# NVIDIA/makani

Measured on AMD Instinct MI355X. Metric: SFNO train samples/sec at 721x1440x73ch, higher is better.
Workload: dtype bf16; 1 GPU; sfno_sc3_layers8_edim384; grid=721x1440, channels=73, global_batch=1, parallelism=dp1, spectral_arithmetic=x3, multistep_count=1, multistep_checkpoint=False, launch=hipGraph replay of the captured step, channel_gemm=hip (csrc/conv1x1.hip)

## Files before the change

makani_amd/csrc/conv1x1.hip:

```cpp
#include <stdlib.h>
#include <type_traits>

#include "common.h"
#include "conv1x1_plan.h"

#ifndef MK_ASTAT_DIAG
#define MK_ASTAT_DIAG 0
#endif
#if MK_ASTAT_DIAG
__device__ unsigned long long g_astat_diag[16];
#define MK_AS_STAMP(k)                                              \
    do {                                                            \
        const unsigned long long t_ = __builtin_readcyclecounter(); \
        dg[k] += t_ - tprev;                                        \
        tprev = t_;                                                 \
    } while (0)
#else
#define MK_AS_STAMP(k)
#endif

namespace {

typedef __bf16 bf16x8 __attribute__((ext_vector_type(8)));
typedef __attribute__((address_space(3))) s16x4 lds_s16x4;
// ... 185 lines not shown
        }
    };

    const int s = lane & 15, g1 = (lane >> 4) & 1;
    const int a_off = (wm * WM + l31) * PA + lh * 8;
    const int b_off = (lh * 8 + (s >> 2)) * PB + wn * WN + g1 * 16 + (s & 3) * 4;
    auto compute = [&](int buf) {
        const u16* Ab = As + buf * BM * PA;
        const u16* Bb = Bs + buf * BK * PB;
#pragma unroll
        for (int ks = 0; ks < BK / 16; ++ks) {
            bf16x8 af[TM], bfr[TN];
#pragma unroll
            for (int i = 0; i < TM; ++i)
                af[i] = __builtin_bit_cast(bf16x8, *reinterpret_cast<const s16x8*>(Ab + a_off + i * 32 * PA + ks * 16));
#pragma unroll
            for (int j = 0; j < TN; ++j) {
                const u16* q0 = Bb + b_off + (ks * 16) * PB + j * 32;
                const s16x4 lo = __builtin_amdgcn_ds_read_tr16_b64_v4i16((lds_s16x4*)(q0));
                const s16x4 hi = __builtin_amdgcn_ds_read_tr16_b64_v4i16((lds_s16x4*)(q0 + 4 * PB));
                const s16x8 v = {lo[0], lo[1], lo[2], lo[3], hi[0], hi[1], hi[2], hi[3]};
                bfr[j] = __builtin_bit_cast(bf16x8, v);
            }
#pragma unroll
            for (int i = 0; i < TM; ++i)
#pragma unroll
                for (int j = 0; j < TN; ++j)
                    acc[i][j] = __builtin_amdgcn_mfma_f32_32x32x16_bf16(af[i], bfr[j], acc[i][j], 0, 0, 0);
        }
    };

    const int nk = (p.K + BK - 1) / BK;
    load_tiles(ra[0], rb[0], 0);
    if constexpr (DEPTH == 2) {
        if (nk > 1) load_tiles(ra[1], rb[1], BK);
        store_tiles(ra[0], rb[0], 0);
        __syncthreads();
        for (int kt = 0; kt < nk; kt += 2) {
            if (kt + 2 < nk) load_tiles(ra[0], rb[0], (kt + 2) * BK);
            compute(0);
            if (kt + 1 < nk) store_tiles(ra[1], rb[1], 1);
            __syncthreads();
            if (kt + 1 >= nk) break;
            if (kt + 3 < nk) load_tiles(ra[1], rb[1], (kt + 3) * BK);
            compute(1);
            if (kt + 2 < nk) store_tiles(ra[0], rb[0], 0);
            __syncthreads();
        }
    } else if constexpr (LDSB == 2) {
        store_tiles(ra[0], rb[0], 0);
        __syncthreads();
        for (int kt = 0; kt < nk; ++kt) {
            if (kt + 1 < nk) load_tiles(ra[0], rb[0], (kt + 1) * BK);
            compute(kt & 1);
            if (kt + 1 < nk) store_tiles(ra[0], rb[0], (kt & 1) ^ 1);
            __syncthreads();
        }
    } else {
        store_tiles(ra[0], rb[0], 0);
        __syncthreads();
        for (int kt = 0; kt < nk; ++kt) {
            if (kt + 1 < nk) load_tiles(ra[0], rb[0], (kt + 1) * BK);
            compute(0);
            __syncthreads();
            if (kt + 1 < nk) {
                store_tiles(ra[0], rb[0], 0);
                __syncthreads();
            }
        }
    }

    const long long plane = (long long)b * p.M * p.N;
    const bool vec_ok = (p.N % 8) == 0;
#pragma unroll
    for (int half = 0; half < 2; ++half) {
        if (wm == half) {
#pragma unroll
            for (int i = 0; i < TM; ++i)
#pragma unroll
                for (int j = 0; j < TN; ++j)
#pragma unroll
                    for (int r = 0; r < 16; ++r) {
                        const int row = i * 32 + (r & 3) + 8 * (r >> 2) + 4 * lh;
                        Es[row * PE + wn * WN + j * 32 + l31] = acc[i][j][r];
                    }
        }
        __syncthreads();
        for (int f = tid; f < WM * (BN / 8); f += NT) {
            const int row = f / (BN / 8), c = f % (BN / 8);
            const int m = m0 + half * WM + row;
            const long long n = n0 + c * 8;
            if (m >= p.M || n >= p.N) continue;
            const float bv = p.bias ? p.bias[m] : 0.f;
            const long long o = plane + (long long)m * p.N + n;
            float v[8];
            const float4 e0 = *reinterpret_cast<const float4*>(Es + row * PE + c * 8);
            const float4 e1 = *reinterpret_cast<const float4*>(Es + row * PE + c * 8 + 4);
            v[0] = e0.x + bv, v[1] = e0.y + bv, v[2] = e0.z + bv, v[3] = e0.w + bv;
            v[4] = e1.x + bv, v[5] = e1.y + bv, v[6] = e1.z + bv, v[7] = e1.w + bv;
            const bool full = vec_ok && n + 8 <= p.N;
            auto put = [&](u16* dst, const float* x) {
                if (full) {
                    uint4 u;
                    u.x = pack_bf16x2(x[0], x[1]);
                    u.y = pack_bf16x2(x[2], x[3]);
                    u.z = pack_bf16x2(x[4], x[5]);
                    u.w = pack_bf16x2(x[6], x[7]);
                    *reinterpret_cast<uint4*>(dst + o) = u;
                } else {
                    for (int e = 0; e < 8 && n + e < p.N; ++e) dst[o + e] = f32_to_bf16(x[e]);
                }
            };
            auto get = [&](const u16* src, float* x) {
                if (full) {
                    const uint4 u = ld16(src + o);
                    const uint32_t w[4] = {u.x, u.y, u.z, u.w};
#pragma unroll
                    for (int e = 0; e < 4; ++e) {
                        x[2 * e] = __uint_as_float(w[e] << 16);
                        x[2 * e + 1] = __uint_as_float(w[e] & 0xffff0000u);
                    }
                } else {
                    for (int e = 0; e < 8; ++e) x[e] = (n + e < p.N) ? bf16_to_f32(src[o + e]) : 0.f;
                }
            };
            if (p.act) {
                if (p.Ypre) put(p.Ypre, v);
#pragma unroll
                for (int e = 0; e < 8; ++e) v[e] = gelu_f(v[e]);
            }
            if (p.G) {
                float g[8];
                get(p.G, g);
#pragma unroll
                for (int e = 0; e < 8; ++e) v[e] *= gelu_grad_f(g[e]);
            }
            if (p.R) {
                float rr[8];
                get(p.R, rr);
#pragma unroll
                for (int e = 0; e < 8; ++e) v[e] += rr[e];
            }
            put(p.Y, v);
        }
        __syncthreads();
    }
}

template <int TM>
__global__ __launch_bounds__(512, 2) void conv_nn_ring_kernel(const ConvNN p, int tilesM, long long tilesN, long long ntiles) {
#if defined(__HIP_DEVICE_COMPILE__)
    constexpr int TN = 2;
    constexpr int BM = 2 * TM * 32, BN = 256, BK = 64;
    constexpr int ASZ = BM * 128, XSZ = BK * BN * 2, STAGE = ASZ + XSZ;
    constexpr int NIA = BM / 64, NIX = 4, NI = NIA + NIX;
    constexpr int EROWS = 64;
    __shared__ __attribute__((aligned(1024))) unsigned char smem[2 * STAGE + EROWS * 512];
    unsigned char* const stg = smem + 2 * STAGE;

    const int tid = threadIdx.x, lane = tid & 63, wave = tid >> 6;
    const int wm = wave >> 2, wn = wave & 3;
    const int l31 = lane & 31, lh = lane >> 5;
    const int nk = (p.K + BK - 1) / BK;
    const unsigned rowbytes = (unsigned)(p.N * 2);

    const int ca_log = (lane & 7) ^ ((((wave & 1) << 2) + (lane >> 4)) & 7);
    const int kx3 = (2 * (wave & 1) + (lane >> 5)) & 3;
    const int cx_log = (lane & 31) ^ (kx3 << 2);
    unsigned voffx[NIX];
#pragma unroll
    for (int j = 0; j < NIX; ++j) voffx[j] = (unsigned)(2 * (wave + 8 * j) + (lane >> 5)) * rowbytes + (unsigned)cx_log * 16u;
    const v4i_t rsA = make_rsrc_n(p.A, (unsigned)((long long)p.M * p.lda * 2));
    const unsigned lds_w = lds_addr(smem) + __builtin_amdgcn_readfirstlane(wave) * 1024;

    const int swa = (l31 >> 1) & 7;
    int aoff[4];
#pragma unroll
    for (int ks = 0; ks < 4; ++ks) aoff[ks] = (wm * TM * 32 + l31) * 128 + (((ks * 2 + lh) ^ swa) * 16);
    const int s15 = lane & 15, g1 = (lane >> 4) & 1;
    int xoff[TN];
#pragma unroll
    for (int j = 0; j < TN; ++j)
        xoff[j] = ASZ + (lh * 8 + (s15 >> 2)) * 512 + ((((wn * TN + j) ^ ((s15 >> 2) & 3)) * 4 + g1 * 2 + ((s15 & 3) >> 1)) * 16) + (s15 & 1) * 8;

    const long long first = xcd_remap(blockIdx.x, gridDim.x);
    unsigned voffa[NIA];
    unsigned voffx_t[NIX];
    const u16* xb = p.X;
    int m0 = 0, bcur = -1;
    long long n0 = 0;

    auto setup_tile = [&](long long t) {
        const int tm = (int)(t % tilesM);
        const long long tnb = t / tilesM;
        const int b = (int)(tnb / tilesN);
        m0 = tm * BM;
        n0 = (tnb % tilesN) * BN;
        if (b != bcur) {
            bcur = b;
            xb = p.X + (long long)b * p.K * p.N;
        }
#pragma unroll
        for (int i = 0; i < NIA; ++i) {
            const int row = min(m0 + (wave + 8 * i) * 8 + (lane >> 3), p.M - 1);
            voffa[i] = (unsigned)row * (unsigned)(p.lda * 2) + (unsigned)ca_log * 16u;
        }
        const int cmax = (int)((min(p.N, n0 + BN) - n0) / 8) - 1;
#pragma unroll
        for (int j = 0; j < NIX; ++j) voffx_t[j] = voffx[j] - (unsigned)max(0, cx_log - cmax) * 16u;
    };
    auto issue = [&](int kt, int stage) {
        const unsigned dst = lds_w + stage * STAGE;
        const unsigned soffa = (unsigned)(kt * BK * 2);
        const v4i_t rsX = make_rsrc_n(xb + (long long)kt * BK * p.N, (unsigned)min(BK, p.K - kt * BK) * rowbytes);
        const unsigned soffx = (unsigned)__builtin_amdgcn_readfirstlane((int)(unsigned)(n0 * 2));
        if constexpr (NIA == 4) dma4<8192>(dst, rsA, soffa, voffa[0], voffa[1], voffa[2], voffa[3]);
        else dma3<8192>(dst, rsA, soffa, voffa[0], voffa[1], voffa[2]);
        dma4<8192>(dst + ASZ, rsX, soffx, voffx_t[0], voffx_t[1], voffx_t[2], voffx_t[3]);
    };

    f32x16 acc[TM][TN];
    auto compute = [&](int stage) {
        const unsigned char* sb = smem + stage * STAGE;
#pragma unroll
        for (int ks = 0; ks < 4; ++ks) {
            bf16x8 af[TM], xf[TN];
#pragma unroll
            for (int i = 0; i < TM; ++i) af[i] = __builtin_bit_cast(bf16x8, *reinterpret_cast<const s16x8*>(sb + aoff[ks] + i * 4096));
#pragma unroll
            for (int j = 0; j < TN; ++j) {
                const unsigned char* q0 = sb + xoff[j] + ks * 16 * 512;
                const s16x4 lo = __builtin_amdgcn_ds_read_tr16_b64_v4i16((lds_s16x4*)(q0));
                const s16x4 hi = __builtin_amdgcn_ds_read_tr16_b64_v4i16((lds_s16x4*)(q0 + 4 * 512));
                const s16x8 v = {lo[0], lo[1], lo[2], lo[3], hi[0], hi[1], hi[2], hi[3]};
                xf[j] = __builtin_bit_cast(bf16x8, v);
            }
#pragma unroll
            for (int i = 0; i < TM; ++i)
#pragma unroll
                for (int j = 0; j < TN; ++j)
                    acc[i][j] = __builtin_amdgcn_mfma_f32_32x32x16_bf16(xf[j], af[i], acc[i][j], 0, 0, 0);
        }
    };

    long long t = first;
    if (t < ntiles) {
        setup_tile(t);
        issue(0, 0);
        if (nk > 1) issue(1, 1);
    }
    for (; t < ntiles; t += gridDim.x) {
#pragma unroll
        for (int i = 0; i < TM; ++i)
#pragma unroll
            for (int j = 0; j < TN; ++j)
#pragma unroll
                for (int r = 0; r < 16; ++r) acc[i][j][r] = 0.f;
        const int cm0 = m0;
        const long long cn0 = n0;
        const int cb = bcur;
        float bvr[TM];
#pragma unroll
        for (int i = 0; i < TM; ++i) {
            const int mrow = cm0 + (wm * TM + i) * 32 + l31;
            bvr[i] = (p.bias && mrow < p.M) ? p.bias[mrow] : 0.f;
        }
#pragma unroll
        for (int i = 0; i < TM; ++i) asm volatile("" : "+v"(bvr[i]));
        for (int kt = 0; kt < nk; ++kt) {
            if (kt == 0 || kt + 1 >= nk) wait_vmcnt<0>(); else wait_vmcnt<NI>();
            __builtin_amdgcn_s_barrier();
            compute(kt & 1);
            asm volatile("s_waitcnt lgkmcnt(0)" ::: "memory");
            __builtin_amdgcn_s_barrier();
            if (kt + 2 < nk) issue(kt + 2, kt & 1);
        }
        const bool have_next = t + gridDim.x < ntiles;
        const bool epi_loads = p.G || p.R;
        if (have_next) setup_tile(t + gridDim.x);
        if (have_next && !epi_loads) {
            issue(0, 0);
            if (nk > 1) issue(1, 1);
        }

        const long long plane = (long long)cb * p.M * p.N;
#pragma unroll
        for (int i = 0; i < TM; ++i) {
            long long off[4];
            bool live[4];
            uint4 gq[4], rq[4];
#pragma unroll
            for (int u4 = 0; u4 < 4; ++u4) {
                const int idx = tid + 512 * u4;
                const int row = idx >> 5, ch = idx & 31;
                const int m = cm0 + ((row >> 5) * TM + i) * 32 + (row & 31);
                const long long n = cn0 + ch * 8;
                live[u4] = m < p.M && n < p.N;
                off[u4] = plane + (long long)m * p.N + n;
                gq[u4] = rq[u4] = make_uint4(0, 0, 0, 0);
                if (live[u4] && p.G) gq[u4] = ld16(p.G + off[u4]);
                if (live[u4] && p.R) rq[u4] = ld16(p.R + off[u4]);
            }
            const float bv = bvr[i];
            const int lrow = wm * 32 + l31;
#pragma unroll
            for (int j = 0; j < TN; ++j)
#pragma unroll
                for (int q = 0; q < 4; ++q) {
                    const int px = (wn * TN + j) * 32 + 8 * q + 4 * lh;
                    uint2 u;
                    u.x = pack_bf16x2(acc[i][j][4 * q] + bv, acc[i][j][4 * q + 1] + bv);
                    u.y = pack_bf16x2(acc[i][j][4 * q + 2] + bv, acc[i][j][4 * q + 3] + bv);
                    *reinterpret_cast<uint2*>(stg + lrow * 512 + (((px >> 3) ^ (lrow & 15)) * 16) + ((px >> 2) & 1) * 8) = u;
                }
            asm volatile("s_waitcnt lgkmcnt(0)" ::: "memory");
            __builtin_amdgcn_s_barrier();
            if (epi_loads) {
#pragma unroll
                for (int u4 = 0; u4 < 4; ++u4) {
                    asm volatile("" : "+v"(gq[u4].x), "+v"(gq[u4].y), "+v"(gq[u4].z), "+v"(gq[u4].w));
                    asm volatile("" : "+v"(rq[u4].x), "+v"(rq[u4].y), "+v"(rq[u4].z), "+v"(rq[u4].w));
                }
                if (i == TM - 1 && have_next) {
                    issue(0, 0);
                    if (nk > 1) issue(1, 1);
                }
            }
#pragma unroll
            for (int u4 = 0; u4 < 4; ++u4) {
                const int idx = tid + 512 * u4;
                const int row = idx >> 5, ch = idx & 31;
                const uint4 raw = *reinterpret_cast<const uint4*>(stg + row * 512 + ((ch ^ (row & 15)) * 16));
                if (live[u4]) {
                    const long long o = off[u4];
                    if (!p.act && !p.G && !p.R) {
                        mk_st16(p.Y + o, raw, p.nt);
                    } else {
                        if (p.act && p.Ypre) mk_st16(p.Ypre + o, raw, p.nt);
                        const uint32_t w[4] = {raw.x, raw.y, raw.z, raw.w};
                        float v[8];
#pragma unroll
                        for (int e = 0; e < 4; ++e) {
                            v[2 * e] = __uint_as_float(w[e] << 16);
                            v[2 * e + 1] = __uint_as_float(w[e] & 0xffff0000u);
                        }
                        if (p.act) {
                            gelu_fast_n<8>(v);
                        }
                        if (p.G) {
                            const uint32_t gw[4] = {gq[u4].x, gq[u4].y, gq[u4].z, gq[u4].w};
#pragma unroll
                            for (int e = 0; e < 4; ++e) {
                                const float ga2[2] = {__uint_as_float(gw[e] << 16), __uint_as_float(gw[e] & 0xffff0000u)};
                                float gd2[2];
                                gelu_grad_fast_n<2>(ga2, gd2);
                                v[2 * e] *= gd2[0];
                                v[2 * e + 1] *= gd2[1];
                            }
                        }
                        if (p.R) {
                            const uint32_t rw[4] = {rq[u4].x, rq[u4].y, rq[u4].z, rq[u4].w};
#pragma unroll
                            for (int e = 0; e < 4; ++e) {
                                v[2 * e] += __uint_as_float(rw[e] << 16);
                                v[2 * e + 1] += __uint_as_float(rw[e] & 0xffff0000u);
                            }
                        }
                        uint4 out;
                        out.x = pack_bf16x2(v[0], v[1]);
                        out.y = pack_bf16x2(v[2], v[3]);
                        out.z = pack_bf16x2(v[4], v[5]);
                        out.w = pack_bf16x2(v[6], v[7]);
                        mk_st16(p.Y + o, out, p.nt);
                    }
                }
            }
            asm volatile("s_waitcnt lgkmcnt(0)" ::: "memory");
            __builtin_amdgcn_s_barrier();
        }
    }
#endif
}

template <int N_> __device__ __forceinline__ void wait_vmcnt_le() {
    if constexpr (N_ <= 63) wait_vmcnt<N_>(); else wait_vmcnt<63>();
}

template <int TM, int KCH, bool PRE, bool EPI_LOADS, int KS = 24>
__global__ __launch_bounds__(256, (KS < 24 && !EPI_LOADS) ? 2 : 1) void conv_nn_astat_kernel(const ConvNN p, int slabs, long long tilesN) {
#if defined(__HIP_DEVICE_COMPILE__)
    constexpr bool SMALLK = KS < 24;
    static_assert(KS == 24 || (KS * 16 <= KCH && KCH % 32 == 0), "small K: one chunk per pixel tile");
    constexpr int TN = 2;
    constexpr int BM = 4 * TM * 32, BN = 64, NT_ = 256;
    constexpr int CH = KCH * 128;
    constexpr int NCH = SMALLK ? 1 : 384 / KCH;
    constexpr int K4 = KS / NCH;
    constexpr int ROUNDS_ = TM;
    constexpr int EBYTES = EPI_LOADS ? ROUNDS_ * 128 * 128 : 0;
    constexpr int NSLOT = SMALLK ? (EPI_LOADS ? 8 : 5) : (EPI_LOADS ? (144 * 1024 - EBYTES) : 128 * 1024) / CH;
    constexpr int NP = KCH / 32;
    constexpr int ROUNDS = TM;
    constexpr int NSTORE = ROUNDS * 4 * (PRE ? 2 : 1);
    constexpr int EPIECES = EPI_LOADS ? ROUNDS * 4 : 0;
    constexpr int LOOK = SMALLK ? ((PRE || EPI_LOADS) ? 2 : 3) : (KCH == 64 ? 8 : ((NP * 4 + 2 * NSTORE <= 63) ? 5 : 4));
    constexpr int SMALLK_EPI_WAIT = NSTORE + (LOOK - 1) * (EPIECES + NP + NSTORE);
    static_assert(!(SMALLK && EPI_LOADS) || SMALLK_EPI_WAIT <= 63, "vmcnt is a 6-bit counter");
    constexpr int NEPI_MAX = (LOOK + NCH - 1) / NCH;
    static_assert(LOOK <= NSLOT - 1, "a slot is refilled only after every wave has left it");
    static_assert(EPI_LOADS || NP * (LOOK - 1) + NEPI_MAX * NSTORE <= 63, "vmcnt is a 6-bit counter");
    __shared__ __attribute__((aligned(1024))) unsigned char smem[NSLOT * CH + EBYTES + 128 * 128];
    unsigned char* const ebuf = smem + NSLOT * CH;
    unsigned char* const stg = ebuf + EBYTES;

    const int tid = threadIdx.x, lane = tid & 63, wave = tid >> 6;
    const bool nt_st = p.nt != 0;
    const int l31 = lane & 31, lh = lane >> 5;
    const int s15 = lane & 15, g1 = (lane >> 4) & 1;
#if MK_ASTAT_DIAG
    unsigned long long dg[8] = {0, 0, 0, 0, 0, 0, 0, 0};
    unsigned long long tprev = __builtin_readcyclecounter();
    const unsigned long long tstart = tprev;
#endif

    const int vid = xcd_remap(blockIdx.x, gridDim.x);
    const int slab = vid % slabs;
    const int pstride = gridDim.x / slabs;
    const int pfirst = vid / slabs;
    const int tilesN32 = (int)tilesN;
    const int my_tiles = pfirst < tilesN32 ? (tilesN32 - pfirst + pstride - 1) / pstride : 0;
    const int cb = blockIdx.y;
    const int m_base = slab * BM + wave * (TM * 32);
    const unsigned nbytes = (unsigned)(p.N * 2);

    bf16x8 af[TM][KS];
#pragma unroll
    for (int i = 0; i < TM; ++i) {
        const int row = min(m_base + i * 32 + l31, p.M - 1);
        const u16* src = p.A + (long long)row * p.lda + lh * 8;
#pragma unroll
        for (int ks = 0; ks < KS; ++ks) af[i][ks] = __builtin_bit_cast(bf16x8, ld16(src + ks * 16));
    }
    float bvr[TM];
#pragma unroll
    for (int i = 0; i < TM; ++i) {
        const int mrow = m_base + i * 32 + l31;
        bvr[i] = (p.bias && mrow < p.M) ? p.bias[mrow] : 0.f;
    }
#pragma unroll
    for (int i = 0; i < TM; ++i) {
#pragma unroll
        for (int ks = 0; ks < KS; ++ks) asm volatile("" : "+v"(af[i][ks]));
        asm volatile("" : "+v"(bvr[i]));
    }

    const unsigned lds0 = lds_addr(smem) + __builtin_amdgcn_readfirstlane(wave) * (NP * 1024);
    unsigned vx[NP];
    const int cxl = (lane & 7) ^ ((((lane >> 3) >> 1) & 1) << 2);
#pragma unroll
    for (int q = 0; q < NP; ++q) vx[q] = (unsigned)((wave * NP + q) * 8 + (lane >> 3)) * nbytes + (unsigned)cxl * 16u;
    const v4i_t rsX = SMALLK ? make_rsrc_n(p.X + (long long)cb * p.K * p.N, (unsigned)p.K * nbytes) : make_rsrc(p.X + (long long)cb * p.K * p.N);
    const unsigned kstride = (unsigned)KCH * nbytes;
    int i_pt = pfirst, i_kc = 0, i_slot = 0;
    auto issue_next = [&]() {
        const unsigned n0b = (unsigned)i_pt * (BN * 2);
        const int cmax = min(7, (int)((nbytes - n0b) / 16) - 1);
        const unsigned soff = (unsigned)__builtin_amdgcn_readfirstlane((int)((unsigned)i_kc * kstride + n0b));
        const unsigned back = (unsigned)max(0, cxl - cmax) * 16u;
        if constexpr (NP == 2) dma2<1024>(lds0 + (unsigned)i_slot * CH, rsX, soff, vx[0] - back, vx[1] - back);
        else if constexpr (NP == 3) dma3<1024>(lds0 + (unsigned)i_slot * CH, rsX, soff, vx[0] - back, vx[1] - back, vx[2] - back);
        else dma4<1024>(lds0 + (unsigned)i_slot * CH, rsX, soff, vx[0] - back, vx[1] - back, vx[2] - back, vx[3] - back);
        i_slot = i_slot + 1 == NSLOT ? 0 : i_slot + 1;
        if (++i_kc == NCH) {
            i_kc = 0;
            i_pt += pstride;
        }
    };

    const u16* const eop = p.G ? p.G : p.R;
    const v4i_t rsE = make_rsrc(EPI_LOADS ? (const void*)(eop + (long long)cb * p.M * p.N) : (const void*)p.X);
    const unsigned ldsE = lds_addr(ebuf) + __builtin_amdgcn_readfirstlane(wave) * 4096;
    auto issue_epi = [&](long long cn0) {
        const unsigned n0b = (unsigned)(cn0 * 2);
        const int cmax = min(7, (int)((nbytes - n0b) / 16) - 1);
        const unsigned col = (unsigned)min(lane & 7, cmax) * 16u;
        const unsigned soff = (unsigned)__builtin_amdgcn_readfirstlane((int)n0b);
#pragma unroll
        for (int i = 0; i < (EPI_LOADS ? ROUNDS_ : 0); ++i) {
            unsigned v[4];
#pragma unroll
            for (int q = 0; q < 4; ++q) v[q] = (unsigned)min(m_base + i * 32 + q * 8 + (lane >> 3), p.M - 1) * nbytes + col;
            dma4<1024>(ldsE + (unsigned)i * 16384u, rsE, soff, v[0], v[1], v[2], v[3]);
        }
    };

    int xoff[TN];
#pragma unroll
    for (int j = 0; j < TN; ++j) {
        const int kk = lh * 8 + (s15 >> 2);
        const int chunk = (j * 4 + g1 * 2 + ((s15 & 3) >> 1)) ^ (((kk >> 1) & 1) << 2);
        xoff[j] = kk * 128 + chunk * 16 + (s15 & 1) * 8;
    }

    const int nchunks = my_tiles * NCH;
    MK_AS_STAMP(7);
    for (int c = 0; c < LOOK && c < nchunks; ++c) issue_next();
    int c_slot = 0;

    f32x16 acc[TM][TN];
    const long long plane0 = (long long)cb * p.M * p.N;
    const __amdgpu_buffer_rsrc_t rsY = __builtin_amdgcn_make_buffer_rsrc((void*)(p.Y + plane0), 0, 0x80000000u, 0x00020000);
    const __amdgpu_buffer_rsrc_t rsP = __builtin_amdgcn_make_buffer_rsrc((void*)((PRE ? p.Ypre : p.Y) + plane0), 0, 0x80000000u, 0x00020000);

    for (int ts = 0; ts < my_tiles; ++ts) {
#pragma unroll
        for (int i = 0; i < TM; ++i)
#pragma unroll
            for (int j = 0; j < TN; ++j)
#pragma unroll
                for (int r = 0; r < 16; ++r) acc[i][j][r] = 0.f;
        const long long cn0 = (long long)(pfirst + ts * pstride) * BN;

#pragma unroll
        for (int kc = 0; kc < NCH; ++kc) {
            const int c = ts * NCH + kc;
            const int nfull = (LOOK - kc + NCH - 1) / NCH;
            if (c + LOOK > nchunks) {
                wait_vmcnt<0>();
            } else if (SMALLK && EPI_LOADS) {
                if (ts < LOOK) wait_vmcnt<0>(); else wait_vmcnt_le<SMALLK_EPI_WAIT>();
            } else if (EPI_LOADS) {
                if (ts < NEPI_MAX) {
// ... 693 lines not shown
    int pa[4], qa[4];
#pragma unroll
    for (int ks = 0; ks < 4; ++ks) {
        const int ch = ((ks * 2 + lh) ^ swz) * 16;
        pa[ks] = (wp * WTP * 32 + l31) * 128 + ch;
        qa[ks] = (TP + wq * WTQ * 32 + l31) * 128 + ch;
    }

    f32x16 acc[WTP][WTQ];
#pragma unroll
    for (int i = 0; i < WTP; ++i)
#pragma unroll
        for (int j = 0; j < WTQ; ++j)
#pragma unroll
            for (int r = 0; r < 16; ++r) acc[i][j][r] = 0.f;

    constexpr int WTG = SWAP ? WTQ : WTP;
    constexpr int NSH = 1;
    const int bshare = 0;
    const bool bias_wave = p.bias_part != nullptr && (SWAP ? (wp == 0 && slab == 0) : (wq == 0 && qs == 0));
    float rsum[WTG];
#pragma unroll
    for (int i = 0; i < WTG; ++i) rsum[i] = 0.f;
    typedef __bf16 bf16x2_t __attribute__((ext_vector_type(2)));
    auto add8 = [](float s, bf16x8 v) {
        const bf16x2_t one = {(__bf16)1.0f, (__bf16)1.0f};
        s = __builtin_amdgcn_fdot2_f32_bf16(bf16x2_t{v[0], v[1]}, one, s, false);
        s = __builtin_amdgcn_fdot2_f32_bf16(bf16x2_t{v[2], v[3]}, one, s, false);
        s = __builtin_amdgcn_fdot2_f32_bf16(bf16x2_t{v[4], v[5]}, one, s, false);
        return __builtin_amdgcn_fdot2_f32_bf16(bf16x2_t{v[6], v[7]}, one, s, false);
    };

    auto compute = [&](int stage) {
        const unsigned char* sb = smem + stage * STAGE;
#pragma unroll
        for (int ks = 0; ks < 4; ++ks) {
            bf16x8 pf[WTP], qf[WTQ];
#pragma unroll
            for (int i = 0; i < WTP; ++i) pf[i] = __builtin_bit_cast(bf16x8, *reinterpret_cast<const s16x8*>(sb + pa[ks] + i * 4096));
#pragma unroll
            for (int j = 0; j < WTQ; ++j) qf[j] = __builtin_bit_cast(bf16x8, *reinterpret_cast<const s16x8*>(sb + qa[ks] + j * 4096));
            if (bias_wave && (ks & (NSH - 1)) == bshare) {
#pragma unroll
                for (int i = 0; i < WTG; ++i) rsum[i] = add8(rsum[i], SWAP ? qf[i] : pf[i]);
            }
#pragma unroll
            for (int i = 0; i < WTP; ++i)
#pragma unroll
                for (int j = 0; j < WTQ; ++j)
                    acc[i][j] = SWAP ? __builtin_amdgcn_mfma_f32_32x32x16_bf16(qf[j], pf[i], acc[i][j], 0, 0, 0)
                                     : __builtin_amdgcn_mfma_f32_32x32x16_bf16(pf[i], qf[j], acc[i][j], 0, 0, 0);
        }
    };

    if (nk > 0) issue(0, 0);
    if (nk > 1) issue(1, 1);
    for (int kt = 0; kt < nk; ++kt) {
        if (kt + 1 < nk) wait_vmcnt<NI>(); else wait_vmcnt<0>();
        __builtin_amdgcn_s_barrier();
        compute(kt & 1);
        asm volatile("s_waitcnt lgkmcnt(0)" ::: "memory");
        __builtin_amdgcn_s_barrier();
        if (kt + 2 < nk) issue(kt + 2, kt & 1);
    }

    if (bias_wave) {
        const int RG = SWAP ? p.RQ : p.RP;
#pragma unroll
        for (int i = 0; i < WTG; ++i) {
            const float tot = rsum[i] + __shfl_xor(rsum[i], 32);
            const int m = SWAP ? q0 + (wq * WTQ + i) * 32 + l31 : slab * TP + (wp * WTP + i) * 32 + l31;
            if (lh == 0 && m < RG) p.bias_part[((long long)sp * NSH + bshare) * RG + m] = tot;
        }
    }

    float* out = p.part + (long long)sp * ((long long)(SWAP ? p.RQ : p.RP) * p.ldo);
#pragma unroll
    for (int i = 0; i < WTP; ++i)
#pragma unroll
        for (int j = 0; j < WTQ; ++j) {
            const int prow0 = slab * TP + (wp * WTP + i) * 32, qrow0 = q0 + (wq * WTQ + j) * 32;
#pragma unroll
            for (int r = 0; r < 16; ++r) {
                const int rr = (r & 3) + 8 * (r >> 2) + 4 * lh;
                const int m = SWAP ? qrow0 + rr : prow0 + rr;
                const int k = SWAP ? prow0 + l31 : qrow0 + l31;
                const bool ok = SWAP ? (m < p.RQ && k < p.RP) : (m < p.RP && k < p.RQ);
                if (ok) out[(long long)m * p.ldo + k] = acc[i][j][r];
            }
        }
#endif
}

__global__ void reduce_splits(const float* __restrict__ part, float* __restrict__ out, long long n, int S, int accumulate) {
    const long long i = (long long)blockIdx.x * blockDim.x + threadIdx.x;
    if (i >= n) return;
    float s = accumulate ? out[i] : 0.f;
    int k = 0;
    for (; k + 8 <= S; k += 8) {
        float v[8];
#pragma unroll
        for (int u = 0; u < 8; ++u) v[u] = part[(long long)(k + u) * n + i];
#pragma unroll
        for (int u = 0; u < 8; ++u) s += v[u];
    }
    for (; k < S; ++k) s += part[(long long)k * n + i];
    out[i] = s;
}

__global__ void reduce_splits4(const float4* __restrict__ part, float4* __restrict__ out, long long n4, int S, int accumulate) {
    const long long i = (long long)blockIdx.x * blockDim.x + threadIdx.x;
    if (i >= n4) return;
    float4 s = accumulate ? out[i] : make_float4(0.f, 0.f, 0.f, 0.f);
    int k = 0;
    for (; k + 8 <= S; k += 8) {
        float4 v[8];
#pragma unroll
        for (int u = 0; u < 8; ++u) v[u] = part[(long long)(k + u) * n4 + i];
#pragma unroll
        for (int u = 0; u < 8; ++u) s.x += v[u].x, s.y += v[u].y, s.z += v[u].z, s.w += v[u].w;
    }
    for (; k < S; ++k) {
        const float4 v = part[(long long)k * n4 + i];
        s.x += v.x, s.y += v.y, s.z += v.z, s.w += v.w;
    }
    out[i] = s;
}

}

#if MK_ASTAT_DIAG
extern "C" int mk_astat_diag_read(unsigned long long* out, int reset) {
    if (hipMemcpyFromSymbol(out, HIP_SYMBOL(g_astat_diag), sizeof(unsigned long long) * 16) != hipSuccess) return 1;
    if (reset) {
        unsigned long long z[16] = {};
        if (hipMemcpyToSymbol(HIP_SYMBOL(g_astat_diag), z, sizeof(z)) != hipSuccess) return 1;
    }
    return 0;
}
#endif

static int env_int(const char* name) {
    const char* e = getenv(name);
    return e ? atoi(e) : -1;
}

extern "C" int mk_conv1x1_nn(const void* A, const void* X, void* Y, void* Ypre, const float* bias, const void* R,
                             const void* G, int M, int K, int lda, int B, long long N, int act, void* stream) {
    MK_REQUIRE(A && X && Y, "conv1x1_nn: null pointer");
    MK_REQUIRE(M > 0 && K > 0 && B > 0 && N > 0, "conv1x1_nn: bad shape M=%d K=%d B=%d N=%lld", M, K, B, N);
    MK_REQUIRE((lda % 8) == 0 && lda >= K, "conv1x1_nn: lda=%d must be a multiple of 8 and >= K=%d", lda, K);
    MK_REQUIRE((N % 8) == 0, "conv1x1_nn: pixel count %lld must be a multiple of 8", N);
    MK_REQUIRE((((uintptr_t)A | (uintptr_t)X) & 15) == 0, "conv1x1_nn: operands must be 16-byte aligned");
    static const int nt_env = env_int("MAKANI_AMD_CONV_NT"), astat2_env = env_int("MAKANI_AMD_ASTAT2");
    const long long out_bytes = (long long)B * M * N * 2;
    const int nt = nt_env == 0 ? 0 : (nt_env == 1 ? 1 : out_bytes <= (256ll << 20));
    ConvNN p{(const u16*)A, (const u16*)X, (u16*)Y, (u16*)Ypre, bias, (const u16*)R, (const u16*)G, M, K, lda, B, N, act, nt};
    hipStream_t s = (hipStream_t)stream;
    const bool pre = act && Ypre, epi_loads = R || G;
    const int slabs = (M + 383) / 384;
    const long long tn64 = (N + 63) / 64;
    auto stationary_grid = [&](int wgs) {
        const long long streams = tn64 < wgs / slabs ? tn64 : wgs / slabs;
        return dim3((unsigned)(streams * slabs), (unsigned)B);
    };
    switch (conv_nn_plan(M, K, lda, B, N, pre, R != nullptr, G != nullptr, astat2_env)) {
    case ConvNnKernel::astat73: {
        const dim3 grid = stationary_grid(epi_loads ? 256 : 512), blk(256);
        if (epi_loads) hipLaunchKernelGGL((conv_nn_astat_kernel<3, 96, false, true, 5>), grid, blk, 0, s, p, slabs, tn64);
        else if (pre) hipLaunchKernelGGL((conv_nn_astat_kernel<3, 96, true, false, 5>), grid, blk, 0, s, p, slabs, tn64);
        else hipLaunchKernelGGL((conv_nn_astat_kernel<3, 96, false, false, 5>), grid, blk, 0, s, p, slabs, tn64);
        break;
    }
    case ConvNnKernel::astat2: {
        const dim3 grid = stationary_grid(256), blk(512);
        if (epi_loads && pre) hipLaunchKernelGGL((conv_nn_astat2_kernel<true, true>), grid, blk, 0, s, p, slabs, tn64);
        else if (epi_loads) hipLaunchKernelGGL((conv_nn_astat2_kernel<false, true>), grid, blk, 0, s, p, slabs, tn64);
        else if (pre) hipLaunchKernelGGL((conv_nn_astat2_kernel<true, false>), grid, blk, 0, s, p, slabs, tn64);
        else hipLaunchKernelGGL((conv_nn_astat2_kernel<false, false>), grid, blk, 0, s, p, slabs, tn64);
        break;
    }
    case ConvNnKernel::astat1: {
        const dim3 grid = stationary_grid(256), blk(256);
#define MK_ASTAT(TM_, KCH_)                                                                                              \
    do {                                                                                                                  \
        if (epi_loads && pre) hipLaunchKernelGGL((conv_nn_astat_kernel<TM_, KCH_, true, true>), grid, blk, 0, s, p, slabs, tn64);   \
        else if (epi_loads) hipLaunchKernelGGL((conv_nn_astat_kernel<TM_, KCH_, false, true>), grid, blk, 0, s, p, slabs, tn64);    \
        else if (pre) hipLaunchKernelGGL((conv_nn_astat_kernel<TM_, KCH_, true, false>), grid, blk, 0, s, p, slabs, tn64);          \
        else hipLaunchKernelGGL((conv_nn_astat_kernel<TM_, KCH_, false, false>), grid, blk, 0, s, p, slabs, tn64);                  \
    } while (0)
        if (epi_loads) MK_ASTAT(3, 64);
        else MK_ASTAT(3, 128);
#undef MK_ASTAT
        break;
    }
    case ConvNnKernel::ring: {
        const bool big = (M % 256 == 0) || M > 576;
        const int bm = big ? 256 : 192;
        const int tm = (M + bm - 1) / bm;
        const long long tn = (N + 255) / 256;
        const long long nt = (long long)tm * tn * B;
        const unsigned grid = (unsigned)(nt < 256 ? nt : 256);
        if (big) hipLaunchKernelGGL((conv_nn_ring_kernel<4>), dim3(grid), dim3(512), 0, s, p, tm, tn, nt);
        else hipLaunchKernelGGL((conv_nn_ring_kernel<3>), dim3(grid), dim3(512), 0, s, p, tm, tn, nt);
        break;
    }
    case ConvNnKernel::tile: {
        constexpr int BM = 128;
        const int tm = (M + BM - 1) / BM;
        const int BN = N >= (1ll << 19) ? 256 : 128;
        const long long tn = (N + BN - 1) / BN;
        const long long nb = (long long)tm * tn * B;
        MK_REQUIRE(nb < (1ll << 31), "conv1x1_nn: grid too large");
        if (BN == 256) hipLaunchKernelGGL((conv_nn_kernel<BM, 256, 1, 64, 2>), dim3((unsigned)nb), dim3(NT), 0, s, p, tm, tn);
        else hipLaunchKernelGGL((conv_nn_kernel<BM, 128, 1, 64, 3>), dim3((unsigned)nb), dim3(NT), 0, s, p, tm, tn);
        break;
    }
    }
    return mk_check_launch("mk_conv1x1_nn");
}

namespace {
struct WgPlan {
    bool ring;
    bool swap;
    int tp;
    int slabs;
    int qslabs;
    long long S;
    long long chunk;
};

WgPlan wgrad_plan(int M, int K, int B, long long N) {
    WgPlan pl{};
    const int big = M > K ? M : K, small = M > K ? K : M;
    if (big >= 96 && N * 2 * 384 < (1ll << 31) && N >= 2048) {
        pl.ring = true;
        int q, pr;
        if (big <= 384) { q = big; pr = small; }
        else if (small <= 384) { q = small; pr = big; }
        else { q = big; pr = small; }
        const bool q_is_x = (K == q) && !(M == q && M > K);
        pl.swap = !q_is_x;
        pl.tp = (pr > 192 && pr % 256 != 192 && (pr % 192 != 0 || pr % 256 == 0)) ? 256 : 192;
        if (pr <= 192) pl.tp = 192;
        pl.slabs = (pr + pl.tp - 1) / pl.tp;
        pl.qslabs = (q + 383) / 384;
        long long per_b = 256 / ((long long)pl.slabs * pl.qslabs * B);
        if (per_b < 1) per_b = 1;
        const long long maxs = (N + 511) / 512;
        if (per_b > maxs) per_b = maxs;
        long long chunk = ((N + per_b - 1) / per_b + 63) / 64 * 64;
        per_b = (N + chunk - 1) / chunk;
        pl.chunk = chunk;
        pl.S = per_b * B;
        return pl;
    }
    const int tiles = ((M + 127) / 128) * ((K + 127) / 128);
    long long per_b = 1024 / ((long long)tiles * B);
    if (per_b < 1) per_b = 1;
    const long long maxs = (N + 2047) / 2048;
    if (per_b > maxs) per_b = maxs;
    long long chunk = (N + per_b - 1) / per_b;
    chunk = (chunk + 127) / 128 * 128;
    pl.chunk = chunk;
    pl.S = per_b * B;
    return pl;
}
}

extern "C" long long mk_conv1x1_wgrad_workspace(int M, int K, int B, long long N) {
    const WgPlan pl = wgrad_plan(M, K, B, N);
    return pl.S * (long long)M * K + pl.S * (long long)M;
}

extern "C" int mk_conv1x1_wgrad_fuses_bias(int M, int K, int B, long long N) {
    return wgrad_plan(M, K, B, N).ring ? 1 : 0;
}

static int conv1x1_wgrad_impl(const void* G, const void* X, float* dW, float* dbias, float* part, int M, int K, int B, long long N,
                              int accumulate, void* stream);

extern "C" int mk_conv1x1_wgrad(const void* G, const void* X, float* dW, float* part, int M, int K, int B, long long N,
                                int accumulate, void* stream) {
    return conv1x1_wgrad_impl(G, X, dW, nullptr, part, M, K, B, N, accumulate, stream);
}

extern "C" int mk_conv1x1_wgrad_bias(const void* G, const void* X, float* dW, float* dbias, float* part, int M, int K, int B,
                                     long long N, int accumulate, void* stream) {
    MK_REQUIRE(dbias, "conv1x1_wgrad_bias: null pointer");
    MK_REQUIRE(wgrad_plan(M, K, B, N).ring, "conv1x1_wgrad_bias: this shape runs the tile kernel, which does not form the bias gradient");
    return conv1x1_wgrad_impl(G, X, dW, dbias, part, M, K, B, N, accumulate, stream);
}

static int conv1x1_wgrad_impl(const void* G, const void* X, float* dW, float* dbias, float* part, int M, int K, int B, long long N,
                              int accumulate, void* stream) {
    MK_REQUIRE(G && X && dW && part, "conv1x1_wgrad: null pointer");
    MK_REQUIRE(M > 0 && K > 0 && B > 0 && N > 0 && (N % 8) == 0, "conv1x1_wgrad: bad shape");
    const WgPlan pl = wgrad_plan(M, K, B, N);
    hipStream_t s = (hipStream_t)stream;
    if (pl.ring) {
        ConvWgR p{};
        p.P = (const u16*)(pl.swap ? X : G);
        p.Q = (const u16*)(pl.swap ? G : X);
        p.RP = pl.swap ? K : M;
        p.RQ = pl.swap ? M : K;
        p.part = part, p.B = B, p.S = (int)pl.S, p.slabs = pl.slabs, p.qslabs = pl.qslabs, p.ldo = K, p.N = N, p.chunk = pl.chunk;
        p.bias_part = dbias ? part + pl.S * (long long)M * K : nullptr;
        const dim3 grid((unsigned)(pl.slabs * pl.qslabs * pl.S)), blk(512);
        if (pl.tp == 256) {
            if (pl.swap) hipLaunchKernelGGL((conv_wgrad_ring_kernel<2, 4, 4, 3, true>), grid, blk, 0, s, p);
            else hipLaunchKernelGGL((conv_wgrad_ring_kernel<2, 4, 4, 3, false>), grid, blk, 0, s, p);
        } else {
            if (pl.swap) hipLaunchKernelGGL((conv_wgrad_ring_kernel<2, 4, 3, 3, true>), grid, blk, 0, s, p);
            else hipLaunchKernelGGL((conv_wgrad_ring_kernel<2, 4, 3, 3, false>), grid, blk, 0, s, p);
        }
    } else {
        const int tm = (M + 127) / 128, tk = (K + 127) / 128;
        ConvWg p{(const u16*)G, (const u16*)X, part, M, K, B, (int)pl.S, N, pl.chunk};
        hipLaunchKernelGGL(conv_wgrad_kernel<128>, dim3((unsigned)(tm * tk * pl.S)), dim3(NT), 0, s, p, tm, tk);
    }
    const long long n = (long long)M * K;
    if (n % 4 == 0 && (((uintptr_t)part | (uintptr_t)dW) & 15) == 0)
        hipLaunchKernelGGL(reduce_splits4, dim3((unsigned)((n / 4 + 255) / 256)), dim3(256), 0, s, (const float4*)part, (float4*)dW,
                           n / 4, (int)pl.S, accumulate);
    else
        hipLaunchKernelGGL(reduce_splits, dim3((unsigned)((n + 255) / 256)), dim3(256), 0, s, part, dW, n, (int)pl.S, accumulate);
    if (dbias)
        hipLaunchKernelGGL(reduce_splits, dim3((unsigned)((M + 255) / 256)), dim3(256), 0, s, part + pl.S * n, dbias, (long long)M,
                           (int)pl.S, 0);
    return mk_check_launch("mk_conv1x1_wgrad");
}
```

makani_amd/csrc/conv1x1_plan.h:

```cpp
#pragma once

enum class ConvNnKernel {
    astat73,
    astat2,
    astat1,
    ring,
    tile
};

inline ConvNnKernel conv_nn_plan(int M, int K, int lda, int B, long long N, bool pre, bool has_r, bool has_g, int astat2_env) {
    const bool stationary = M >= 256 && (long long)M * N * 2 < (1ll << 31) && N >= 64 && !(has_r && has_g);
    if (stationary && lda == 80 && K > 64 && K <= 80 && (long long)K * N * 2 < (1ll << 32) && !((has_r || has_g) && pre))
        return ConvNnKernel::astat73;
    const bool small_ring = M == 384 && (long long)B * N <= 32768 && !pre && astat2_env != 1;
    if (stationary && K == 384 && !small_ring) return astat2_env == 0 ? ConvNnKernel::astat1 : ConvNnKernel::astat2;
    if (K >= 64 && M >= 192 && N * 2 * 64 < (1ll << 31) && (long long)M * lda * 2 < (1ll << 31) && N >= 256) return ConvNnKernel::ring;
    return ConvNnKernel::tile;
}
```

Baseline: 27.13 samples/s.

## Add 384-row ring GEMM tile variant for M<=384 plain channel GEMMs

Adds a TM=6 instantiation of the ring conv1x1 kernel that covers a whole 384-row weight block per tile, so each pixel tile of X is loaded once instead of twice. To fit LDS, the epilogue staging buffer aliases stage 0 of the weight buffer, and the next tile's prefetch is split so the aliased part is issued only after the epilogue finishes. Register pressure is reduced by recomputing DMA offsets and loading bias after the K loop. It is enabled by default only for K>=512, M in (192,384], no epilogue inputs, and enough tiles. The risks are higher register pressure and less prefetch overlap at tile boundaries.

Measured after the change: 27.69 samples/s, median of 6. 1.02x the previous value.

```diff
diff --git a/makani_amd/csrc/conv1x1.hip b/makani_amd/csrc/conv1x1.hip
--- a/makani_amd/csrc/conv1x1.hip
+++ b/makani_amd/csrc/conv1x1.hip
@@ -361,13 +361,21 @@
 #if defined(__HIP_DEVICE_COMPILE__)
     constexpr int TN = 2;
     constexpr int BM = 2 * TM * 32, BN = 256, BK = 64;
+    constexpr bool WIDE = TM == 6;
     constexpr int ASZ = BM * 128, XSZ = BK * BN * 2, STAGE = ASZ + XSZ;
     constexpr int NIA = BM / 64, NIX = 4, NI = NIA + NIX;
     constexpr int EROWS = 64;
-    __shared__ __attribute__((aligned(1024))) unsigned char smem[2 * STAGE + EROWS * 512];
-    unsigned char* const stg = smem + 2 * STAGE;
+    static_assert(!WIDE || EROWS * 512 == 4 * 8192, "the staging image covers the first four weight row groups of stage 0");
+    __shared__ __attribute__((aligned(1024))) unsigned char smem[2 * STAGE + (WIDE ? 0 : EROWS * 512)];
+    unsigned char* const stg = WIDE ? smem : smem + 2 * STAGE;
 
     const int tid = threadIdx.x, lane = tid & 63, wave = tid >> 6;
+    const int wv = WIDE ? __builtin_amdgcn_readfirstlane(wave) : wave;
+    auto lane_here = [&]() __attribute__((always_inline)) {
+        int l = lane;
+        asm volatile("" : "+v"(l));
+        return l;
+    };
     const int wm = wave >> 2, wn = wave & 3;
     const int l31 = lane & 31, lh = lane >> 5;
     const int nk = (p.K + BK - 1) / BK;
@@ -398,6 +406,7 @@
     const u16* xb = p.X;
     int m0 = 0, bcur = -1;
     long long n0 = 0;
+    int cmax_t = 0;
 
     auto setup_tile = [&](long long t) {
         const int tm = (int)(t % tilesM);
@@ -409,36 +418,57 @@
             bcur = b;
             xb = p.X + (long long)b * p.K * p.N;
         }
-#pragma unroll
-        for (int i = 0; i < NIA; ++i) {
-            const int row = min(m0 + (wave + 8 * i) * 8 + (lane >> 3), p.M - 1);
-            voffa[i] = (unsigned)row * (unsigned)(p.lda * 2) + (unsigned)ca_log * 16u;
-        }
-        const int cmax = (int)((min(p.N, n0 + BN) - n0) / 8) - 1;
-#pragma unroll
-        for (int j = 0; j < NIX; ++j) voffx_t[j] = voffx[j] - (unsigned)max(0, cx_log - cmax) * 16u;
-    };
-    auto issue = [&](int kt, int stage) {
+        if constexpr (WIDE) {
+            cmax_t = (int)((min(p.N, n0 + BN) - n0) / 8) - 1;
+        } else {
+#pragma unroll
+            for (int i = 0; i < NIA; ++i) {
+                const int row = min(m0 + (wave + 8 * i) * 8 + (lane >> 3), p.M - 1);
+                voffa[i] = (unsigned)row * (unsigned)(p.lda * 2) + (unsigned)ca_log * 16u;
+            }
+            const int cmax = (int)((min(p.N, n0 + BN) - n0) / 8) - 1;
+#pragma unroll
+            for (int j = 0; j < NIX; ++j) voffx_t[j] = voffx[j] - (unsigned)max(0, cx_log - cmax) * 16u;
+        }
+    };
+    auto issue = [&](int kt, int stage, int part = 0) __attribute__((always_inline)) {
         const unsigned dst = lds_w + stage * STAGE;
         const unsigned soffa = (unsigned)(kt * BK * 2);
         const v4i_t rsX = make_rsrc_n(xb + (long long)kt * BK * p.N, (unsigned)min(BK, p.K - kt * BK) * rowbytes);
         const unsigned soffx = (unsigned)__builtin_amdgcn_readfirstlane((int)(unsigned)(n0 * 2));
-        if constexpr (NIA == 4) dma4<8192>(dst, rsA, soffa, voffa[0], voffa[1], voffa[2], voffa[3]);
-        else dma3<8192>(dst, rsA, soffa, voffa[0], voffa[1], voffa[2]);
-        dma4<8192>(dst + ASZ, rsX, soffx, voffx_t[0], voffx_t[1], voffx_t[2], voffx_t[3]);
+        if constexpr (WIDE) {
+            const int ln = lane_here();
+            const unsigned ca16 = (unsigned)((ln & 7) ^ ((((wv & 1) << 2) + (ln >> 4)) & 7)) * 16u;
+            const int row0 = m0 + wv * 8 + (ln >> 3);
+            auto va = [&](int i) { return (unsigned)min(row0 + 64 * i, p.M - 1) * (unsigned)(p.lda * 2) + ca16; };
+            if (part != 1) dma4<8192>(dst, rsA, soffa, va(0), va(1), va(2), va(3));
+            if (part != 2) {
+                dma2<8192>(dst + 4 * 8192, rsA, soffa, va(4), va(5));
+                const int cx = (ln & 31) ^ (((2 * (wv & 1) + (ln >> 5)) & 3) << 2);
+                const unsigned vx = (unsigned)(2 * wv + (ln >> 5)) * rowbytes + (unsigned)min(cx, cmax_t) * 16u, r16 = 16u * rowbytes;
+                dma4<8192>(dst + ASZ, rsX, soffx, vx, vx + r16, vx + 2 * r16, vx + 3 * r16);
+            }
+        } else {
+            if constexpr (NIA == 4) dma4<8192>(dst, rsA, soffa, voffa[0], voffa[1], voffa[2], voffa[3]);
+            else dma3<8192>(dst, rsA, soffa, voffa[0], voffa[1], voffa[2]);
+            dma4<8192>(dst + ASZ, rsX, soffx, voffx_t[0], voffx_t[1], voffx_t[2], voffx_t[3]);
+        }
     };
 
     f32x16 acc[TM][TN];
     auto compute = [&](int stage) {
         const unsigned char* sb = smem + stage * STAGE;
+        int a0 = aoff[0], x0 = xoff[0];
+        if constexpr (WIDE) asm volatile("" : "+v"(a0), "+v"(x0));
 #pragma unroll
         for (int ks = 0; ks < 4; ++ks) {
             bf16x8 af[TM], xf[TN];
-#pragma unroll
-            for (int i = 0; i < TM; ++i) af[i] = __builtin_bit_cast(bf16x8, *reinterpret_cast<const s16x8*>(sb + aoff[ks] + i * 4096));
+            const int ao = WIDE ? (a0 ^ (ks * 32)) : aoff[ks];
+#pragma unroll
+            for (int i = 0; i < TM; ++i) af[i] = __builtin_bit_cast(bf16x8, *reinterpret_cast<const s16x8*>(sb + ao + i * 4096));
 #pragma unroll
             for (int j = 0; j < TN; ++j) {
-                const unsigned char* q0 = sb + xoff[j] + ks * 16 * 512;
+                const unsigned char* q0 = sb + (WIDE ? (x0 ^ (j * 64)) : xoff[j]) + ks * 16 * 512;
                 const s16x4 lo = __builtin_amdgcn_ds_read_tr16_b64_v4i16((lds_s16x4*)(q0));
                 const s16x4 hi = __builtin_amdgcn_ds_read_tr16_b64_v4i16((lds_s16x4*)(q0 + 4 * 512));
                 const s16x8 v = {lo[0], lo[1], lo[2], lo[3], hi[0], hi[1], hi[2], hi[3]};
@@ -469,13 +499,16 @@
         const long long cn0 = n0;
         const int cb = bcur;
         float bvr[TM];
-#pragma unroll
-        for (int i = 0; i < TM; ++i) {
-            const int mrow = cm0 + (wm * TM + i) * 32 + l31;
-            bvr[i] = (p.bias && mrow < p.M) ? p.bias[mrow] : 0.f;
-        }
-#pragma unroll
-        for (int i = 0; i < TM; ++i) asm volatile("" : "+v"(bvr[i]));
+        auto fetch_bias = [&]() __attribute__((always_inline)) {
+#pragma unroll
+            for (int i = 0; i < TM; ++i) {
+                const int mrow = cm0 + (wm * TM + i) * 32 + l31;
+                bvr[i] = (p.bias && mrow < p.M) ? p.bias[mrow] : 0.f;
+            }
+#pragma unroll
+            for (int i = 0; i < TM; ++i) asm volatile("" : "+v"(bvr[i]));
+        };
+        if constexpr (!WIDE) fetch_bias();
         for (int kt = 0; kt < nk; ++kt) {
             if (kt == 0 || kt + 1 >= nk) wait_vmcnt<0>(); else wait_vmcnt<NI>();
             __builtin_amdgcn_s_barrier();
@@ -484,11 +517,12 @@
             __builtin_amdgcn_s_barrier();
             if (kt + 2 < nk) issue(kt + 2, kt & 1);
         }
+        if constexpr (WIDE) fetch_bias();
         const bool have_next = t + gridDim.x < ntiles;
-        const bool epi_loads = p.G || p.R;
+        const bool epi_loads = !WIDE && (p.G || p.R);
         if (have_next) setup_tile(t + gridDim.x);
         if (have_next && !epi_loads) {
-            issue(0, 0);
+            issue(0, 0, WIDE ? 1 : 0);
             if (nk > 1) issue(1, 1);
         }
 
@@ -507,8 +541,8 @@
                 live[u4] = m < p.M && n < p.N;
                 off[u4] = plane + (long long)m * p.N + n;
                 gq[u4] = rq[u4] = make_uint4(0, 0, 0, 0);
-                if (live[u4] && p.G) gq[u4] = ld16(p.G + off[u4]);
-                if (live[u4] && p.R) rq[u4] = ld16(p.R + off[u4]);
+                if (!WIDE && live[u4] && p.G) gq[u4] = ld16(p.G + off[u4]);
+                if (!WIDE && live[u4] && p.R) rq[u4] = ld16(p.R + off[u4]);
             }
             const float bv = bvr[i];
             const int lrow = wm * 32 + l31;
@@ -542,7 +576,7 @@
                 const uint4 raw = *reinterpret_cast<const uint4*>(stg + row * 512 + ((ch ^ (row & 15)) * 16));
                 if (live[u4]) {
                     const long long o = off[u4];
-                    if (!p.act && !p.G && !p.R) {
+                    if (WIDE || (!p.act && !p.G && !p.R)) {
                         mk_st16(p.Y + o, raw, p.nt);
                     } else {
                         if (p.act && p.Ypre) mk_st16(p.Ypre + o, raw, p.nt);
@@ -587,6 +621,7 @@
             asm volatile("s_waitcnt lgkmcnt(0)" ::: "memory");
             __builtin_amdgcn_s_barrier();
         }
+        if (WIDE && have_next && !epi_loads) issue(0, 0, 2);
     }
 #endif
 }
@@ -1586,7 +1621,8 @@
     MK_REQUIRE((lda % 8) == 0 && lda >= K, "conv1x1_nn: lda=%d must be a multiple of 8 and >= K=%d", lda, K);
     MK_REQUIRE((N % 8) == 0, "conv1x1_nn: pixel count %lld must be a multiple of 8", N);
     MK_REQUIRE((((uintptr_t)A | (uintptr_t)X) & 15) == 0, "conv1x1_nn: operands must be 16-byte aligned");
-    static const int nt_env = env_int("MAKANI_AMD_CONV_NT"), astat2_env = env_int("MAKANI_AMD_ASTAT2");
+    static const int nt_env = env_int("MAKANI_AMD_CONV_NT"), astat2_env = env_int("MAKANI_AMD_ASTAT2"),
+                     ring384_env = env_int("MAKANI_AMD_RING384");
     const long long out_bytes = (long long)B * M * N * 2;
     const int nt = nt_env == 0 ? 0 : (nt_env == 1 ? 1 : out_bytes <= (256ll << 20));
     ConvNN p{(const u16*)A, (const u16*)X, (u16*)Y, (u16*)Ypre, bias, (const u16*)R, (const u16*)G, M, K, lda, B, N, act, nt};
@@ -1629,13 +1665,13 @@
         break;
     }
     case ConvNnKernel::ring: {
-        const bool big = (M % 256 == 0) || M > 576;
-        const int bm = big ? 256 : 192;
+        const int bm = conv_nn_ring_rows(M, K, B, N, act || Ypre || R || G, ring384_env);
         const int tm = (M + bm - 1) / bm;
         const long long tn = (N + 255) / 256;
         const long long nt = (long long)tm * tn * B;
         const unsigned grid = (unsigned)(nt < 256 ? nt : 256);
-        if (big) hipLaunchKernelGGL((conv_nn_ring_kernel<4>), dim3(grid), dim3(512), 0, s, p, tm, tn, nt);
+        if (bm == 384) hipLaunchKernelGGL((conv_nn_ring_kernel<6>), dim3(grid), dim3(512), 0, s, p, tm, tn, nt);
+        else if (bm == 256) hipLaunchKernelGGL((conv_nn_ring_kernel<4>), dim3(grid), dim3(512), 0, s, p, tm, tn, nt);
         else hipLaunchKernelGGL((conv_nn_ring_kernel<3>), dim3(grid), dim3(512), 0, s, p, tm, tn, nt);
         break;
     }
diff --git a/makani_amd/csrc/conv1x1_plan.h b/makani_amd/csrc/conv1x1_plan.h
--- a/makani_amd/csrc/conv1x1_plan.h
+++ b/makani_amd/csrc/conv1x1_plan.h
@@ -17,3 +17,10 @@
     if (K >= 64 && M >= 192 && N * 2 * 64 < (1ll << 31) && (long long)M * lda * 2 < (1ll << 31) && N >= 256) return ConvNnKernel::ring;
     return ConvNnKernel::tile;
 }
+
+inline int conv_nn_ring_rows(int M, int K, int B, long long N, bool has_epilogue, int ring384_env) {
+    const int rows = ((M % 256 == 0) || M > 576) ? 256 : 192;
+    const long long tiles384 = ((N + 255) / 256) * B;
+    if (rows == 192 && M > 192 && M <= 384 && K >= 512 && !has_epilogue && tiles384 >= 256 && ring384_env != 0) return 384;
+    return rows;
+}
```
